# mycophonic/saprobe-alac

Hardware: AMD Instinct MI355X
Metric: Msamples/s decoded (16-bit stereo, 4096-frame packets) (higher is better)
Workload: dtype int32; 1 GPU; 65536 packets/GPU x 16-bit 2-ch 4096-frame ALAC, music-like synthetic, device-resident in/out; packets_per_gpu=65536

## Files before the change

### saprobe-alac_amd/csrc/alac_gpu.h

```cpp
#ifndef ALAC_GPU_H
#define ALAC_GPU_H
#include <hip/hip_runtime.h>

#include <algorithm>
#include <cstdio>
#include <cstdlib>
#include <cstring>

#define ALAC_DEV __device__ __forceinline__
#define ALAC_HD __host__ __device__ __forceinline__
#define ALAC_NOINLINE
#define ALAC_MUL24(a, b) __mul24((int)(a), (int)(b))
__device__ __forceinline__ uint32_t alac_sad(uint32_t a, uint32_t b, uint32_t c) {
    uint32_t r;
    asm("v_sad_u32 %0, %1, %2, %3" : "=v"(r) : "v"(a), "v"(b), "v"(c));
    return r;
}
#define ALAC_SAD(a, b, c) alac_sad((uint32_t)(a), (uint32_t)(b), (uint32_t)(c))

__device__ __forceinline__ int32_t alac_sign_med3(int32_t x) {
    int32_t r;
    asm("v_med3_i32 %0, %1, -1, 1" : "=v"(r) : "v"(x));
    return r;
}
// ... 102 lines not shown
#include "alac_duo.h"
#include "alac_split.h"

#define ALAC_PRIO_B_LONG 3
#define ALAC_PRIO_B_MID 2
#define ALAC_PRIO_B_SHORT 1
#define ALAC_PRIO_A 2
#define ALAC_PRIO_C 3

namespace alack {


typedef uint32_t u32x4 __attribute__((ext_vector_type(4)));

constexpr uint32_t kWave = 64;
constexpr uint32_t kTimingSlots = 64;
#ifndef ALAC_LDS_ROWS
#define ALAC_LDS_ROWS 64
#endif
#ifndef ALAC_LDS_RING
#define ALAC_LDS_RING 32
#endif
#ifndef ALAC_LDS_FLUSH
#define ALAC_LDS_FLUSH (ALAC_LDS_ROWS / 2)
#endif
constexpr uint32_t kRing = ALAC_LDS_ROWS;
constexpr uint32_t kFlush = ALAC_LDS_FLUSH;
static_assert(kFlush <= kRing && kRing % 4 == 0 && (kFlush == 16 || kFlush == 32), "the stager flushes 64- or 128-byte pieces of its rows");
constexpr uint32_t kRowStride = kRing + 1;
constexpr uint32_t kFallbackSlots = 64;
constexpr uint32_t kRingDw = ALAC_LDS_RING;
constexpr uint32_t kRingSlots = kRingDw + 2;

constexpr uint32_t kKeys = alac::KEY_IRREGULAR + 2u;
constexpr uint32_t kKeyLegacy = alac::KEY_IRREGULAR;
constexpr uint32_t kKeyScan = alac::KEY_IRREGULAR + 1u;
struct Plan {
    uint32_t count[kKeys];
    uint32_t pkt_start[kKeys];
    uint32_t cursor[kKeys];
    uint32_t nk;
    uint32_t list_key[kKeys];
    uint32_t list_wave0[kKeys];
    uint32_t total_waves;
    uint32_t irr_waves;
    uint32_t wide_waves;
    uint32_t gate[2][512];
    uint32_t balance[2][512];
    uint32_t queue[2];
};

static __shared__ uint32_t s_rows[kWave * kRowStride];
static __shared__ unsigned long long s_optr[kWave];
static __shared__ __attribute__((aligned(16))) uint32_t s_ring[kRingSlots * kWave];
constexpr uint32_t kQ = alac::DUO_CHUNK;
static __shared__ int32_t s_rq[2 * kQ * kWave];

#ifdef ALAC_SYNC_DIAG
constexpr uint32_t kClaimDw = 16;
static __shared__ uint32_t s_dg_arrive;
#else
constexpr uint32_t kClaimDw = 4;
#endif

__host__ __device__ inline size_t u_tile_cells(uint32_t frame_length) { return ((size_t)frame_length + 1u) * kWave; }

struct GpuWave {
    static constexpr bool kResMem = false;
    static constexpr uint32_t kRingDw = alack::kRingDw;
    int32_t* u_tile;
    int32_t* g_tile;
    uint8_t* my_out;
    uint32_t lane, wcnt, flushed;
    uint32_t ppw;
#ifdef ALAC_SYNC_DIAG
    uint32_t dg_wait[2] = {0, 0}, dg_last[2] = {0, 0};
    uint32_t dg_phase = 0, dg_waves = 3;
#endif

    ALAC_DEV bool any(bool p) const { return __ballot(p) != 0ull; }
    ALAC_DEV uint32_t max_u32(uint32_t v) const {
#pragma unroll
// ... 144 lines not shown
        asm volatile("s_waitcnt lgkmcnt(0)\n\ts_barrier" ::: "memory");
        dg_wait[dg_phase] += (uint32_t)(__builtin_amdgcn_s_memtime() - t0);
        dg_last[dg_phase] += (old + 1u) % dg_waves == 0u ? 1u : 0u;
    }
#endif
    ALAC_DEV void duo_sync_mem() {
        __threadfence_block();
        __syncthreads();
    }
    ALAC_DEV int32_t* u_row(uint32_t i) const { return u_tile + ((size_t)i * kWave + (ppw < kWave ? (lane < ppw ? lane : ppw) : lane)); }
    ALAC_DEV int32_t* g_slot(uint32_t k) const { return g_tile + (size_t)k * ppw; }
};

struct GpuWaveMem : GpuWave {
    static constexpr bool kResMem = true;
    const int32_t* res;
    uint32_t it, chunk0;
    ALAC_DEV int32_t rq_read(uint32_t, uint32_t j) const { return res[chunk0 + j]; }
    ALAC_DEV void rq_write(uint32_t, uint32_t, int32_t) {}
    ALAC_DEV void duo_sync() {
        ++it;
        chunk0 = (it - 1u) * kQ;
    }
    ALAC_DEV void duo_sync_mem() {}
};

__device__ __forceinline__ uint32_t avail_of(uint64_t blob_bytes, uint64_t off) {
    const uint64_t left = blob_bytes - off;
    return left > 0xffffffffull ? 0xffffffffu : (uint32_t)left;
}

__global__ void alac_classify(alac::DevCfg cfg, const uint8_t* __restrict__ blob, uint64_t blob_bytes, const uint64_t* __restrict__ offsets,
                              const uint32_t* __restrict__ sizes, uint32_t n, uint16_t* __restrict__ keys, uint32_t* __restrict__ sizes_ws,
                              uint32_t* __restrict__ frames_out, int32_t* __restrict__ status, Plan* plan);
__global__ void alac_plan(Plan* plan, uint32_t ppw);
__global__ void alac_cu_census(uint32_t* __restrict__ seen, uint32_t* __restrict__ arrived, uint32_t expect);
__global__ void alac_scatter(const uint16_t* __restrict__ keys, uint32_t n, Plan* plan, uint32_t* __restrict__ perm);
__global__ void alac_task_classify(alac::DevCfg cfg, const alac::ChanDesc* __restrict__ cd, const alac::PktDesc* __restrict__ pd,
                                   const uint16_t* __restrict__ pkt_keys, uint32_t n_slots, uint16_t* __restrict__ keys, Plan* plan);
__global__ void alac_scan(alac::DevCfg cfg, const uint8_t* __restrict__ blob, uint64_t blob_bytes, const uint64_t* __restrict__ offsets,
                          const uint32_t* __restrict__ sizes, const uint32_t* __restrict__ perm, const Plan* __restrict__ plan,
                          uint8_t* __restrict__ out, uint64_t out_stride, uint32_t* __restrict__ frames_out,
                          int32_t* __restrict__ status, int32_t* __restrict__ scratch_u, int32_t* __restrict__ scratch_g,
                          uint32_t ppw, alac::ChanDesc* __restrict__ cd, alac::PktDesc* __restrict__ pd, int32_t* __restrict__ rows,
                          uint64_t row_stride);
__global__ void alac_legacy(alac::DevCfg cfg, const uint8_t* __restrict__ blob, uint64_t blob_bytes, const uint64_t* __restrict__ offsets,
                            const uint32_t* __restrict__ sizes, const uint32_t* __restrict__ perm, const Plan* __restrict__ plan,
                            const alac::PktDesc* __restrict__ pd, uint8_t* __restrict__ out, uint64_t out_stride,
                            uint32_t* __restrict__ frames_out, int32_t* __restrict__ status, int32_t* __restrict__ scratch_u,
                            int32_t* __restrict__ scratch_g, uint32_t ppw);
constexpr uint32_t kModeFit4 = 4u, kModeFit5 = 5u, kModeGated = 6u;
constexpr __host__ __device__ __forceinline__ uint32_t decode_mode(uint32_t items, uint32_t n_cu, uint32_t cap, uint32_t force, bool mono,
                                                                  bool fit5) {
    if (force == kModeFit4 || (force == kModeFit5 && fit5)) return force;
    if (items <= 4u * n_cu) return kModeFit4;
    if (items <= 5u * n_cu) return (cap >= 5u && !mono) ? kModeGated : fit5 ? kModeFit5 : kModeFit4;
    if (items <= 6u * n_cu && cap >= 6u) return kModeGated;
    return (2u * items <= 15u * n_cu || !fit5) ? kModeFit4 : kModeFit5;
}
constexpr __host__ __device__ __forceinline__ uint32_t pair_quota(uint32_t items, uint32_t n_cu, uint32_t cap) {
    const uint32_t need = (items + n_cu - 1u) / n_cu;
    return need < 5u ? 5u : need < cap ? need : cap;
}
constexpr bool mode_is_fit4_without_the_others(uint32_t n_cu) {
    for (uint32_t items = 0u; items <= 40u * n_cu; items += (items < 8u * n_cu ? 1u : n_cu / 2u + 1u))
        if (decode_mode(items, n_cu, 0u, 0u, false, false) != kModeFit4 || decode_mode(items, n_cu, 0u, 5u, true, false) != kModeFit4) return false;
    return true;
}
constexpr bool mode_is_fit4_within_four(uint32_t n_cu) {
    for (uint32_t cap = 0u; cap <= 8u; ++cap)
        for (uint32_t items = 0u; items <= 4u * n_cu; ++items)
            if (decode_mode(items, n_cu, cap, 0u, false, true) != kModeFit4 || decode_mode(items, n_cu, cap, 0u, true, true) != kModeFit4) return false;
// ... 50 lines not shown
```

### saprobe-alac_amd/csrc/alacgpu.hip

```cpp
#include "alac_gpu.h"
#include "alac_host.h"
#include "alac_waveform.h"
#include "alac_clips.h"

using namespace alack;

namespace {
thread_local char g_err[512] = "";
}

void alack::set_err(const char* fmt, ...) {
    va_list ap;
    va_start(ap, fmt);
    vsnprintf(g_err, sizeof(g_err), fmt, ap);
    va_end(ap);
}

namespace {

class CopyPool {
public:
    explicit CopyPool(unsigned threads) {
        for (unsigned t = 0; t < threads; ++t) workers_.emplace_back([this] { run(); });
    }
    ~CopyPool() {
        {
            std::lock_guard<std::mutex> g(m_);
            stop_ = true;
        }
        cv_.notify_all();
        for (auto& w : workers_) w.join();
    }
// ... 90 lines not shown
Kernels choose_kernels(const alac::DevCfg& c) {
    Kernels k{};
    k.lean = alac::lean_config(c);
    k.one_or_two = c.num_channels <= 2;
    k.quad = c.bit_depth == 16 ? ALAC_PAIR_KERNEL(alac_decode_16q) : c.bit_depth == 32 ? ALAC_PAIR_KERNEL(alac_decode_32q) : ALAC_PAIR_KERNEL(alac_decode_24q);
    k.gated = c.bit_depth == 16 ? ALAC_PAIR_KERNEL(alac_decode_16g) : PairKernel{nullptr, ""};
    k.wide = c.bit_depth == 32 ? ALAC_PAIR_KERNEL(alac_decode_w32) : c.bit_depth == 24 ? ALAC_PAIR_KERNEL(alac_decode_w24) : PairKernel{nullptr, ""};
    const bool four_frames = c.num_channels > 2 && (c.num_channels * c.bps) % 4u == 0u;
    k.interleave = four_frames ? alac_interleave4 : alac_interleave;
    k.interleave_lds = (four_frames ? 128u : 32u) * kWave;
    k.irregular = !k.lean        ? "alac_scan (whole-packet decoder)"
                  : k.one_or_two ? "alac_scan + alac_interleave (+ alac_legacy)"
                  : four_frames  ? "alac_scan + alac_chan_predict + alac_interleave4 (+ alac_legacy)"
                                 : "alac_scan + alac_chan_predict + alac_interleave (+ alac_legacy)";
    return k;
}
#undef ALAC_PAIR_KERNEL

}

struct alacgpu_decoder {
    alacgpu_config cfg;
    alac::DevCfg dev_cfg;
    Kernels kernels;
    int device;
    size_t frame_bytes;
    hipStream_t stream;
    hipStream_t s_in, s_out;
    hipStream_t s_side;
    hipEvent_t ev_fork, ev_join;
    hipEvent_t ev_start[kTimingSlots], ev_stop[kTimingSlots];
    uint64_t launches;
    DevBuf scratch_u, scratch_g, plan, cls, perm, sizes_ws;
    DevBuf cd, pd, plan2, keys2, perm2, rows;
    Slot slots[kSlots];
    CopyPool* pool;
    uint32_t n_cu;
    DevBuf cu_number;
    size_t chunk_bytes;
    uint32_t lanes_min;
    int side;
    std::thread* ahead;
    int ahead_rc;
    char ahead_err[512];
    size_t last_n;
    uint32_t last_ppw, last_cap, last_fit5;
    uint32_t fit_force;
    DevBuf wave_ws;
    hipEvent_t ev_w0, ev_w1;
    bool wave_timed;
    hipEvent_t ev_c0, ev_c1;
    bool clips_timed;
};

namespace {

size_t plan_claims_offset() { return (sizeof(Plan) + 255u) & ~(size_t)255u; }
size_t plan_bytes(size_t waves) { return plan_claims_offset() + waves * kClaimDw * sizeof(uint32_t); }

struct KernelAttr {
    uint32_t pairs_per_cu, static_lds;
};
KernelAttr kernel_attr(void (*kernel)(PairArgs)) {
    static std::mutex mu;
    static std::vector<std::pair<const void*, KernelAttr>> cache;
    std::lock_guard<std::mutex> g(mu);
// ... 21 lines not shown
    HIP_TRY(hipMemcpyAsync(seen, dec->cu_number.p, sizeof(seen), hipMemcpyDeviceToHost, dec->stream));
    HIP_TRY(hipStreamSynchronize(dec->stream));
    uint32_t per_xcd[8] = {0}, xcds = 0, total = 0;
    for (uint32_t i = 0; i < 512; i++)
        if (seen[i]) {
            per_xcd[i >> 6]++;
            total++;
        }
    for (uint32_t x = 0; x < 8; x++) xcds += per_xcd[x] ? 1u : 0u;
    if (xcds == 0) xcds = 1;
    uint32_t next[8] = {0}, order[8] = {0}, k = 0;
    for (uint32_t x = 0; x < 8; x++)
        if (per_xcd[x]) order[x] = k++;
    for (uint32_t i = 0; i < 512; i++)
        if (seen[i]) {
            const uint32_t x = i >> 6;
            seen[i] = 1u + next[x]++ * xcds + order[x];
        }
    if (total > dec->n_cu) dec->n_cu = total;
    HIP_TRY(hipMemcpyAsync(dec->cu_number.p, seen, sizeof(seen), hipMemcpyHostToDevice, dec->stream));
    HIP_TRY(hipStreamSynchronize(dec->stream));
    return ALACGPU_E_OK;
}

size_t max_waves(uint32_t bit_depth, size_t n, uint32_t ppw) {
    const size_t keys = (bit_depth >= 24 ? 2 : 1) * 18 * 18 + 8;
    return (n + ppw - 1) / ppw + std::min<size_t>(n, keys);
}
size_t max_waves(const alacgpu_decoder* dec, size_t n, uint32_t ppw) { return max_waves(dec->cfg.bit_depth, n, ppw); }

uint32_t pick_ppw(size_t n) {
    if (const char* e = getenv("ALACGPU_PPW")) {
        const int v = atoi(e);
        if (v >= 1 && v <= 64) return (uint32_t)v;
    }
    uint32_t ppw = kWave;
    while (ppw > 1 && n / ppw < 256) ppw >>= 1;
    return ppw;
}

size_t row_stride_of(uint32_t frame_length) { return ((size_t)frame_length + 3u) & ~(size_t)3u; }

int reserve_workspace(alacgpu_decoder* dec, size_t n, uint32_t ppw) {
    const size_t waves = max_waves(dec, n, ppw);
    int rc;
    if ((rc = dec->scratch_u.ensure(waves * u_tile_cells(dec->cfg.frame_length) * sizeof(int32_t)))) return rc;
    if ((rc = dec->scratch_g.ensure(waves * kFallbackSlots * ppw * sizeof(int32_t)))) return rc;
    if ((rc = dec->plan.ensure(plan_bytes(waves)))) return rc;
    if ((rc = dec->cls.ensure((n ? n : 1) * sizeof(uint16_t)))) return rc;
    if ((rc = dec->perm.ensure((n ? n : 1) * sizeof(uint32_t)))) return rc;
    if ((rc = dec->sizes_ws.ensure((n ? n : 1) * sizeof(uint32_t)))) return rc;
    const size_t ns = (n ? n : 1) * 8;
    if ((rc = dec->cd.ensure(ns * sizeof(alac::ChanDesc)))) return rc;
    if ((rc = dec->pd.ensure((n ? n : 1) * sizeof(alac::PktDesc)))) return rc;
    if (dec->cfg.num_channels > 2) {
        if ((rc = dec->plan2.ensure(sizeof(Plan)))) return rc;
        if ((rc = dec->keys2.ensure(ns * sizeof(uint16_t)))) return rc;
        if ((rc = dec->perm2.ensure(ns * sizeof(uint32_t)))) return rc;
        if ((rc = dec->rows.ensure((n ? n : 1) * dec->cfg.num_channels * row_stride_of(dec->cfg.frame_length) * sizeof(int32_t))))
            return rc;
    }
    return ALACGPU_E_OK;
}

struct Launch {
    alacgpu_decoder* dec;
    alac::DevCfg c;
    const uint8_t* d_blob;
    uint64_t blob_bytes;
    const uint64_t* d_offsets;
    size_t n;
    uint8_t* d_out;
    size_t out_stride;
    uint32_t* d_frames;
    int32_t* d_status;
    uint32_t ppw;
    size_t waves;
    hipStream_t irr;
    bool forked;
    uint32_t scan_grid;
    Plan* plan() const { return (Plan*)dec->plan.p; }
    const uint32_t* sz() const { return (const uint32_t*)dec->sizes_ws.p; }
};

struct SideFork {
    alacgpu_decoder* dec;
    bool open = false;
    int fork() {
        HIP_TRY(hipEventRecord(dec->ev_fork, dec->stream));
        HIP_TRY(hipStreamWaitEvent(dec->s_side, dec->ev_fork, 0));
        open = true;
        return ALACGPU_E_OK;
    }
    int join() {
        HIP_TRY(hipEventRecord(dec->ev_join, dec->s_side));
        HIP_TRY(hipStreamWaitEvent(dec->stream, dec->ev_join, 0));
        open = false;
        return ALACGPU_E_OK;
    }
    ~SideFork() {
        if (open) (void)hipStreamSynchronize(dec->s_side);
    }
};

int sort_pass(const Launch& L, const uint32_t* d_sizes) {
    alacgpu_decoder* dec = L.dec;
    const uint32_t nb = (uint32_t)((L.n + 255) / 256);
    HIP_TRY(hipMemsetAsync(L.plan(), 0, plan_bytes(L.waves), dec->stream));
    hipLaunchKernelGGL(alac_classify, dim3(nb), dim3(256), 0, dec->stream, L.c, L.d_blob, L.blob_bytes, L.d_offsets, d_sizes,
                       (uint32_t)L.n, (uint16_t*)dec->cls.p, (uint32_t*)dec->sizes_ws.p, L.d_frames, L.d_status, L.plan());
    hipLaunchKernelGGL(alac_plan, dim3(1), dim3(kWave), 0, dec->stream, L.plan(), L.ppw);
    hipLaunchKernelGGL(alac_scatter, dim3(nb), dim3(256), 0, dec->stream, (const uint16_t*)dec->cls.p, (uint32_t)L.n, L.plan(),
                       (uint32_t*)dec->perm.p);
    return ALACGPU_E_OK;
}

void scan(const Launch& L) {
    alacgpu_decoder* dec = L.dec;
    hipLaunchKernelGGL(alac_scan, dim3(L.scan_grid), dim3(kWave), 0, L.irr, L.c, L.d_blob, L.blob_bytes,
                       L.d_offsets, L.sz(), (const uint32_t*)dec->perm.p, (const Plan*)L.plan(), L.d_out, (uint64_t)L.out_stride, L.d_frames,
                       L.d_status, (int32_t*)dec->scratch_u.p, (int32_t*)dec->scratch_g.p, L.ppw, (alac::ChanDesc*)dec->cd.p,
                       (alac::PktDesc*)dec->pd.p, dec->cfg.num_channels > 2 ? (int32_t*)dec->rows.p : (int32_t*)nullptr,
                       (uint64_t)row_stride_of(dec->cfg.frame_length));
}

void narrow_launch(const Launch& L, const PairArgs& a, uint32_t slots, uint32_t mode) {
    alacgpu_decoder* dec = L.dec;
    const Kernels& k = dec->kernels;
    if (mode == kModeGated) {
        if (a.cap) hipLaunchKernelGGL(k.gated.fn, dim3(std::min<uint32_t>(a.cap * dec->n_cu, slots)), dim3(2 * kWave), 0, dec->stream, a);
        return;
    }
    if (mode == kModeFit5 && !a.fit5) return;
    const uint32_t stat = kernel_attr(k.quad.fn).static_lds;
    PairArgs q = a;
    q.fit = mode;
    hipLaunchKernelGGL(k.quad.fn, dim3(slots), dim3(4 * kWave), (mode == kModeFit4 && stat < kQuadLdsFit4) ? kQuadLdsFit4 - stat : 0u,
                       dec->stream, q);
}

void regular_packets(const Launch& L) {
    alacgpu_decoder* dec = L.dec;
    const Kernels& k = dec->kernels;
    const size_t n = L.n;
    const uint32_t ppw = L.ppw;
    PairArgs a{L.c, L.d_blob, (uint64_t)L.blob_bytes, L.d_offsets, L.sz(), (const uint32_t*)dec->perm.p, L.plan(), L.d_out, (uint64_t)L.out_stride,
               L.d_frames, L.d_status, (int32_t*)dec->scratch_u.p, (const uint32_t*)dec->cu_number.p,
               (uint32_t*)((uint8_t*)L.plan() + plan_claims_offset()), ppw, dec->n_cu, 0u, dec->lanes_min, 4u, dec->fit_force, 0u};
    const uint32_t slots = (uint32_t)L.waves;
    const uint32_t n_cu = dec->n_cu;
    const bool beyond4 = (n + ppw - 1) / ppw > (size_t)4 * n_cu || dec->fit_force == kModeFit5;
    const bool has_twin = k.gated.fn && beyond4 && dec->fit_force == 0u;
    {
        const uint32_t stat = kernel_attr(k.quad.fn).static_lds;
        a.fit5 = (beyond4 && (size_t)((stat + 1279u) / 1280u) * 1280u * 5u <= 163840u) ? 1u : 0u;
    }
    if (has_twin) a.cap = kernel_attr(k.gated.fn).pairs_per_cu;
    if (a.cap <= 4u) a.cap = 0u;
    dec->last_cap = a.cap;
    dec->last_fit5 = a.fit5;
    const uint32_t guess = decode_mode((uint32_t)((n + ppw - 1) / ppw), n_cu, a.cap, dec->fit_force, dec->cfg.num_channels == 1, a.fit5 != 0u);
    narrow_launch(L, a, slots, guess);
    if (k.wide.fn) hipLaunchKernelGGL(k.wide.fn, dim3(slots), dim3(2 * kWave), 0, dec->stream, a);
    for (uint32_t mode : {kModeFit4, kModeFit5, kModeGated})
        if (mode != guess) narrow_launch(L, a, slots, mode);
}

int split_pipeline(const Launch& L) {
    alacgpu_decoder* dec = L.dec;
    Plan* plan2 = (Plan*)dec->plan2.p;
    const size_t n_slots = L.n * 8;
    const uint32_t nb2 = (uint32_t)((n_slots + 255) / 256);
    const uint32_t ppw2 = pick_ppw(L.n * dec->cfg.num_channels);
    HIP_TRY(hipMemsetAsync(plan2, 0, sizeof(Plan), dec->stream));
    hipLaunchKernelGGL(alac_task_classify, dim3(nb2), dim3(256), 0, dec->stream, L.c, (const alac::ChanDesc*)dec->cd.p,
                       (const alac::PktDesc*)dec->pd.p, (const uint16_t*)dec->cls.p, (uint32_t)n_slots,
                       (uint16_t*)dec->keys2.p, plan2);
    hipLaunchKernelGGL(alac_plan, dim3(1), dim3(kWave), 0, dec->stream, plan2, ppw2);
    hipLaunchKernelGGL(alac_scatter, dim3(nb2), dim3(256), 0, dec->stream, (const uint16_t*)dec->keys2.p,
                       (uint32_t)n_slots, plan2, (uint32_t*)dec->perm2.p);
    hipLaunchKernelGGL(alac_chan_predict, dim3((uint32_t)max_waves(16u, n_slots, ppw2)), dim3(kWave), 0, dec->stream, L.c,
                       L.d_blob, L.blob_bytes, L.d_offsets, L.sz(), (const uint32_t*)dec->perm2.p, (const Plan*)plan2,
                       (const alac::ChanDesc*)dec->cd.p, (int32_t*)dec->rows.p, (uint64_t)row_stride_of(dec->cfg.frame_length), ppw2);
    return ALACGPU_E_OK;
}

void irregular_pcm(const Launch& L) {
    alacgpu_decoder* dec = L.dec;
    const Kernels& k = dec->kernels;
    const uint64_t rs = row_stride_of(dec->cfg.frame_length);
    const uint32_t bpp = (dec->cfg.frame_length + kWave - 1u) / kWave;
    const uint32_t ib = (uint32_t)std::min<uint64_t>((uint64_t)L.n * ((bpp + 7u) / 8u), L.forked ? (uint64_t)4 * dec->n_cu : (uint64_t)32768u);
    hipLaunchKernelGGL(k.interleave, dim3(ib), dim3(kWave), k.interleave_lds, L.irr, L.c, L.d_blob, L.blob_bytes, L.d_offsets, L.sz(),
                       (const uint32_t*)dec->perm.p, (const Plan*)L.plan(), (const alac::ChanDesc*)dec->cd.p,
                       (const alac::PktDesc*)dec->pd.p, (const int32_t*)dec->rows.p, rs, L.d_out, (uint64_t)L.out_stride, bpp);
    hipLaunchKernelGGL(alac_legacy, dim3(L.scan_grid), dim3(kWave), 0, L.irr, L.c, L.d_blob, L.blob_bytes,
                       L.d_offsets, L.sz(), (const uint32_t*)dec->perm.p, (const Plan*)L.plan(), (const alac::PktDesc*)dec->pd.p, L.d_out,
                       (uint64_t)L.out_stride, L.d_frames, L.d_status, (int32_t*)dec->scratch_u.p, (int32_t*)dec->scratch_g.p, L.ppw);
}

int launch(alacgpu_decoder* dec, const uint8_t* d_blob, uint64_t blob_bytes, const uint64_t* d_offsets,
           const uint32_t* d_sizes, size_t n, uint8_t* d_out, size_t out_stride, uint32_t* d_frames, int32_t* d_status) {
    if (n == 0) return ALACGPU_E_OK;
    if (n > 0x7fffffffu) {
        set_err("batch too large");
        return ALACGPU_E_ARG;
    }
    const uint32_t ppw = pick_ppw(n);
    int rc = reserve_workspace(dec, n, ppw);
    if (rc) return rc;
    dec->last_n = n;
    dec->last_ppw = ppw;
    dec->last_cap = dec->last_fit5 = 0;
    const Kernels& k = dec->kernels;
    Launch L{dec, dec->dev_cfg, d_blob, blob_bytes, d_offsets, n, d_out, out_stride, d_frames, d_status, ppw, max_waves(dec, n, ppw),
             dec->stream, false, 0u};
    L.c.aligned16 = (out_stride % 16 == 0 && (reinterpret_cast<uintptr_t>(d_out) % 16) == 0) ? 1u : 0u;
    const uint32_t slot = (uint32_t)(dec->launches % kTimingSlots);
    HIP_TRY(hipEventRecord(dec->ev_start[slot], dec->stream));
    if ((rc = sort_pass(L, d_sizes))) return rc;
    L.forked = k.one_or_two && k.lean &&
               (dec->side >= 2 || (dec->side == 1 && (n + ppw - 1) / ppw <= (size_t)6 * dec->n_cu));
    L.scan_grid = (uint32_t)std::min<size_t>(L.waves, (size_t)(L.forked ? 2u : 6u) * dec->n_cu);
    SideFork side{dec};
    if (L.forked) {
        if ((rc = side.fork())) return rc;
        L.irr = dec->s_side;
    }
    if (!L.forked) scan(L);
    if (k.one_or_two && k.lean) regular_packets(L);
    if (L.forked) scan(L);
    HIP_TRY(hipGetLastError());
    if (k.lean) {
        if (!k.one_or_two && (rc = split_pipeline(L))) return rc;
        irregular_pcm(L);
        HIP_TRY(hipGetLastError());
    }
    if (L.forked && (rc = side.join())) return rc;
    HIP_TRY(hipEventRecord(dec->ev_stop[slot], dec->stream));
    dec->launches++;
    return ALACGPU_E_OK;
}

}

namespace {
std::mutex g_pool_mu;
std::vector<alacgpu_decoder*> g_pool;
std::vector<std::pair<void*, size_t>> g_host_pool;
std::vector<std::pair<void*, size_t>> g_host_sizes;
constexpr size_t kPoolPerDevice = 4;
constexpr size_t kPoolKeepDevice = (size_t)2048 << 20;
constexpr size_t kPoolKeepPinned = (size_t)64 << 20;
constexpr size_t kHostPoolBlock = (size_t)64 << 20, kHostPoolBytes = (size_t)192 << 20, kHostPoolCount = 8;
template <class Buf>
void keep_at_most(std::vector<Buf*> bufs, size_t limit) {
    for (;;) {
        size_t total = 0;
        Buf* big = nullptr;
        for (Buf* b : bufs) {
            total += b->cap;
            if (b->cap && (!big || b->cap > big->cap)) big = b;
        }
        if (total <= limit || !big) return;
        big->release();
    }
}

std::vector<DevBuf*> device_buffers(alacgpu_decoder* d) {
    std::vector<DevBuf*> v = {&d->scratch_u, &d->scratch_g, &d->plan, &d->cls, &d->perm, &d->sizes_ws, &d->cd, &d->pd,
                              &d->plan2, &d->keys2, &d->perm2, &d->rows, &d->wave_ws};
    for (Slot& s : d->slots) v.insert(v.end(), {&s.d_in, &s.d_out});
    return v;
}
std::vector<HostBuf*> pinned_buffers(alacgpu_decoder* d) {
    std::vector<HostBuf*> v;
    for (Slot& s : d->slots) v.insert(v.end(), {&s.h_in, &s.h_out});
    return v;
}
std::vector<hipStream_t*> streams_of(alacgpu_decoder* d) { return {&d->stream, &d->s_in, &d->s_out, &d->s_side}; }
struct EventRef {
    hipEvent_t* ev;
    unsigned flags;
};
std::vector<EventRef> events_of(alacgpu_decoder* d) {
    std::vector<EventRef> v = {{&d->ev_fork, hipEventDisableTiming}, {&d->ev_join, hipEventDisableTiming},
                               {&d->ev_w0, hipEventDefault}, {&d->ev_w1, hipEventDefault},
                               {&d->ev_c0, hipEventDefault}, {&d->ev_c1, hipEventDefault}};
    for (uint32_t i = 0; i < kTimingSlots; i++) v.insert(v.end(), {{&d->ev_start[i], hipEventDefault}, {&d->ev_stop[i], hipEventDefault}});
    for (Slot& s : d->slots)
        v.insert(v.end(), {{&s.ev_in, hipEventDisableTiming}, {&s.ev_k, hipEventDisableTiming}, {&s.ev_out, hipEventDisableTiming}});
    return v;
}

bool synchronize_all(alacgpu_decoder* d) {
    bool ok = true;
    for (hipStream_t* s : streams_of(d))
        if (*s && hipStreamSynchronize(*s) != hipSuccess) ok = false;
    return ok;
}

void really_destroy(alacgpu_decoder* d) {
    (void)hipSetDevice(d->device);
// ... 79 lines not shown
        return ALACGPU_E_ARG;
    }
    d->device = device;
    configure(d, cfg);
    {
        int cus = 0;
        if (hipDeviceGetAttribute(&cus, hipDeviceAttributeMultiprocessorCount, device) != hipSuccess) cus = 0;
        d->n_cu = cus > 0 ? (uint32_t)cus : 256u;
    }
    hipError_t e = hipSuccess;
    for (hipStream_t* st : streams_of(d))
        if (e == hipSuccess) e = hipStreamCreateWithFlags(st, hipStreamNonBlocking);
    for (const EventRef& ev : events_of(d))
        if (e == hipSuccess) e = hipEventCreateWithFlags(ev.ev, ev.flags);
    if (e != hipSuccess) {
        set_err("stream/event creation failed: %s", hipGetErrorString(e));
        really_destroy(d);
        return ALACGPU_E_HIP;
    }
    if (int rc = cu_numbers(d)) {
        really_destroy(d);
        return rc;
    }
    *out = d;
    return ALACGPU_E_OK;
}

void alacgpu_destroy(alacgpu_decoder* d) {
    if (!d) return;
    (void)settle_ahead(d);
    (void)hipSetDevice(d->device);
    if (synchronize_all(d)) {
        for (int k = 0; k < kSlots; k++) d->slots[k].busy = false;
        keep_at_most(device_buffers(d), kPoolKeepDevice);
        keep_at_most(pinned_buffers(d), kPoolKeepPinned);
        std::lock_guard<std::mutex> g(g_pool_mu);
        size_t same = 0;
        for (alacgpu_decoder* p : g_pool) same += p->device == d->device ? 1u : 0u;
        if (same < kPoolPerDevice) {
            g_pool.push_back(d);
            return;
        }
    }
    really_destroy(d);
}

void alacgpu_trim(void) {
    std::vector<alacgpu_decoder*> all;
    std::vector<std::pair<void*, size_t>> host;
    {
        std::lock_guard<std::mutex> g(g_pool_mu);
        all.swap(g_pool);
        host.swap(g_host_pool);
    }
    for (alacgpu_decoder* d : all) really_destroy(d);
    for (auto& h : host) (void)hipHostFree(h.first);
}

void* alacgpu_host_alloc(size_t bytes) {
    if (bytes == 0) bytes = 1;
    {
        std::lock_guard<std::mutex> g(g_pool_mu);
        size_t best = SIZE_MAX;
        for (size_t i = 0; i < g_host_pool.size(); i++)
            if (g_host_pool[i].second >= bytes && g_host_pool[i].second <= 2 * bytes + (1u << 20) &&
                (best == SIZE_MAX || g_host_pool[i].second < g_host_pool[best].second))
// ... 513 lines not shown
```

### saprobe-alac_amd/csrc/k_sort.hip

```cpp
#include "alac_gpu.h"

namespace alack {

__global__ void __launch_bounds__(256)
alac_classify(alac::DevCfg cfg, const uint8_t* __restrict__ blob, uint64_t blob_bytes, const uint64_t* __restrict__ offsets,
              const uint32_t* __restrict__ sizes, uint32_t n, uint16_t* __restrict__ keys, uint32_t* __restrict__ sizes_ws,
              uint32_t* __restrict__ frames_out, int32_t* __restrict__ status, Plan* plan) {
    __shared__ uint32_t hist[kKeys];
    for (uint32_t k = threadIdx.x; k < kKeys; k += blockDim.x) hist[k] = 0;
    __syncthreads();
    const uint32_t i = blockIdx.x * blockDim.x + threadIdx.x;
    if (i < n) {
        const uint64_t off = offsets[i];
        uint64_t sz = sizes ? (uint64_t)sizes[i] : offsets[i + 1] - off;
        const bool ok = off <= blob_bytes && sz <= blob_bytes - off && sz <= 0x0fffffffull &&
                        (sizes || offsets[i + 1] >= off);
        if (!ok) {
            keys[i] = (uint16_t)alac::TASK_NONE;
            sizes_ws[i] = 0;
            frames_out[i] = 0;
            status[i] = ALACGPU_ERR_RANGE;
        } else if (sz == 0) {
            keys[i] = (uint16_t)alac::TASK_NONE;
            sizes_ws[i] = 0;
            frames_out[i] = 0;
            status[i] = ALACGPU_STATUS(alac::ST_OVERRUN, 0, 0);
        } else {
            sizes_ws[i] = (uint32_t)sz;
            const uint8_t* p = blob + off;
            uint32_t key = alac::classify_regular(cfg, p, (uint32_t)sz, avail_of(blob_bytes, off));
            if (key == alac::KEY_IRREGULAR) key = alac::lean_config(cfg) ? kKeyScan : kKeyLegacy;
            keys[i] = (uint16_t)key;
            atomicAdd(&hist[key], 1u);
        }
    }
    __syncthreads();
    for (uint32_t k = threadIdx.x; k < kKeys; k += blockDim.x)
        if (hist[k]) atomicAdd(&plan->count[k], hist[k]);
}

__global__ void __launch_bounds__(kWave) alac_plan(Plan* plan, uint32_t ppw) {
    __shared__ uint32_t cnt[kKeys];
    for (uint32_t k = threadIdx.x; k < kKeys; k += kWave) cnt[k] = plan->count[k];
    __syncthreads();
    constexpr uint32_t R = (kKeys + kWave - 1) / kWave;
    const uint32_t q0 = threadIdx.x * R;
    uint32_t p = 0, w = 0, z = 0, wi = 0, ww = 0;
    for (uint32_t r = 0; r < R; ++r) {
        const uint32_t q = q0 + r;
        if (q >= kKeys) break;
        const uint32_t key = kKeys - 1u - q;
        const uint32_t c = cnt[key];
        const uint32_t cw = (c + ppw - 1) / ppw;
        p += c;
        w += cw;
        z += c ? 1u : 0u;
        wi += key >= alac::KEY_IRREGULAR ? cw : 0u;
        ww += (key >= alac::KEY_WIDE && key < alac::KEY_IRREGULAR) ? cw : 0u;
    }
    uint32_t ip = p, iw = w, iz = z, ii = wi, ix = ww;
#pragma unroll
    for (int o = 1; o < (int)kWave; o <<= 1) {
        const uint32_t tp = (uint32_t)__shfl_up((int)ip, o, kWave), tw = (uint32_t)__shfl_up((int)iw, o, kWave);
        const uint32_t tz = (uint32_t)__shfl_up((int)iz, o, kWave), ti = (uint32_t)__shfl_up((int)ii, o, kWave);
        const uint32_t tx = (uint32_t)__shfl_up((int)ix, o, kWave);
        if ((int)threadIdx.x >= o) {
            ix += tx;
            ip += tp;
            iw += tw;
            iz += tz;
            ii += ti;
        }
    }
    uint32_t ep = ip - p, ew = iw - w, ez = iz - z;
    for (uint32_t r = 0; r < R; ++r) {
        const uint32_t q = q0 + r;
        if (q >= kKeys) break;
        const uint32_t key = kKeys - 1u - q;
        const uint32_t c = cnt[key];
        plan->pkt_start[key] = ep;
        plan->cursor[key] = 0;
        if (c) {
            plan->list_key[ez] = key;
            plan->list_wave0[ez] = ew;
            ++ez;
            ep += c;
            ew += (c + ppw - 1) / ppw;
        }
    }
    if (threadIdx.x == kWave - 1u) {
        plan->nk = iz;
        plan->total_waves = iw;
        plan->irr_waves = ii;
        plan->wide_waves = ix;
    }
}

__global__ void __launch_bounds__(256)
alac_scatter(const uint16_t* __restrict__ keys, uint32_t n, Plan* plan, uint32_t* __restrict__ perm) {
    __shared__ uint32_t hist[kKeys];
    __shared__ uint32_t base[kKeys];
    for (uint32_t k = threadIdx.x; k < kKeys; k += blockDim.x) hist[k] = 0;
    __syncthreads();
    const uint32_t i = blockIdx.x * blockDim.x + threadIdx.x;
    uint32_t key = 0, local = 0;
    if (i < n) {
        key = keys[i];
        if (key != alac::TASK_NONE) local = atomicAdd(&hist[key], 1u);
    }
    __syncthreads();
    for (uint32_t k = threadIdx.x; k < kKeys; k += blockDim.x)
        if (hist[k]) base[k] = plan->pkt_start[k] + atomicAdd(&plan->cursor[k], hist[k]);
    __syncthreads();
    if (i < n && key != alac::TASK_NONE) perm[base[key] + local] = i;
}

__global__ void __launch_bounds__(256)
alac_task_classify(alac::DevCfg cfg, const alac::ChanDesc* __restrict__ cd, const alac::PktDesc* __restrict__ pd,
                   const uint16_t* __restrict__ pkt_keys, uint32_t n_slots, uint16_t* __restrict__ keys, Plan* plan) {
    __shared__ uint32_t hist[alac::NUM_TASK_KEYS];
    if (threadIdx.x < alac::NUM_TASK_KEYS) hist[threadIdx.x] = 0;
    __syncthreads();
    const uint32_t t = blockIdx.x * blockDim.x + threadIdx.x;
    if (t < n_slots) {
        const uint32_t pkt = t >> 3, slot = t & 7u;
        uint32_t key = alac::TASK_NONE;
        if (pkt_keys[pkt] == kKeyScan) {
            const alac::PktDesc q = pd[pkt];
            if (q.status == 0 && q.route == alac::ROUTE_SPLIT && slot < q.nslots) {
                const alac::ChanDesc d = cd[t];
                if ((d.info & alac::CD_VALID) && !(d.info & alac::CD_ESCAPE)) key = alac::chan_task_key(cfg, d);
            }
        }
        keys[t] = (uint16_t)key;
        if (key != alac::TASK_NONE) atomicAdd(&hist[key], 1u);
    }
    __syncthreads();
    if (threadIdx.x < alac::NUM_TASK_KEYS && hist[threadIdx.x]) atomicAdd(&plan->count[threadIdx.x], hist[threadIdx.x]);
}

__global__ void __launch_bounds__(kWave) alac_cu_census(uint32_t* __restrict__ seen, uint32_t* __restrict__ arrived, uint32_t expect) {
    __shared__ uint32_t pad[16384];
    pad[threadIdx.x] = threadIdx.x;
    if (threadIdx.x == 0) {
        uint32_t id, xcc;
        asm volatile("s_getreg_b32 %0, hwreg(HW_REG_HW_ID)" : "=s"(id));
        asm volatile("s_getreg_b32 %0, hwreg(HW_REG_XCC_ID)" : "=s"(xcc));
        seen[((xcc & 7u) << 6) | (((id >> 13) & 3u) << 4) | ((id >> 8) & 15u)] = 1u;
        atomicAdd(arrived, 1u);
        for (int i = 0; i < 4000 && atomicAdd(arrived, 0u) < expect; ++i) __builtin_amdgcn_s_sleep(32);
    }
    __syncthreads();
    if (pad[(threadIdx.x * 5u) & 63u] == 0xffffffffu) seen[0] = 2u;
}

}
```

Before: 264,200 Msamples/s.

## Fuse plan computation into classify via last-block ticket and rank-based scatter

```diff
diff --git a/saprobe-alac_amd/csrc/alac_gpu.h b/saprobe-alac_amd/csrc/alac_gpu.h
--- a/saprobe-alac_amd/csrc/alac_gpu.h
+++ b/saprobe-alac_amd/csrc/alac_gpu.h
@@ -158,22 +158,13 @@
 constexpr uint32_t kRingDw = ALAC_LDS_RING;
 constexpr uint32_t kRingSlots = kRingDw + 2;
 
-constexpr uint32_t kKeys = alac::KEY_IRREGULAR + 2u;
-constexpr uint32_t kKeyLegacy = alac::KEY_IRREGULAR;
-constexpr uint32_t kKeyScan = alac::KEY_IRREGULAR + 1u;
-struct Plan {
-    uint32_t count[kKeys];
-    uint32_t pkt_start[kKeys];
-    uint32_t cursor[kKeys];
-    uint32_t nk;
-    uint32_t list_key[kKeys];
-    uint32_t list_wave0[kKeys];
-    uint32_t total_waves;
-    uint32_t irr_waves;
-    uint32_t wide_waves;
-    uint32_t gate[2][512];
-    uint32_t balance[2][512];
-    uint32_t queue[2];
+}
+#include "alac_plan.h"
+namespace alack {
+
+struct SortWs {
+    uint32_t hist[kKeys];
+    uint32_t ticket;
 };
 
 static __shared__ uint32_t s_rows[kWave * kRowStride];
@@ -384,12 +375,14 @@
 
 __global__ void alac_classify(alac::DevCfg cfg, const uint8_t* __restrict__ blob, uint64_t blob_bytes, const uint64_t* __restrict__ offsets,
                               const uint32_t* __restrict__ sizes, uint32_t n, uint16_t* __restrict__ keys, uint32_t* __restrict__ sizes_ws,
-                              uint32_t* __restrict__ frames_out, int32_t* __restrict__ status, Plan* plan);
-__global__ void alac_plan(Plan* plan, uint32_t ppw);
+                              uint32_t* __restrict__ frames_out, int32_t* __restrict__ status, uint32_t* __restrict__ rank, SortWs* ws, Plan* plan,
+                              uint32_t ppw_shift);
 __global__ void alac_cu_census(uint32_t* __restrict__ seen, uint32_t* __restrict__ arrived, uint32_t expect);
-__global__ void alac_scatter(const uint16_t* __restrict__ keys, uint32_t n, Plan* plan, uint32_t* __restrict__ perm);
+__global__ void alac_scatter(const uint16_t* __restrict__ keys, const uint32_t* __restrict__ rank, uint32_t n, const Plan* __restrict__ plan,
+                             uint32_t* __restrict__ perm, uint32_t* __restrict__ claims, uint32_t claim_dw);
 __global__ void alac_task_classify(alac::DevCfg cfg, const alac::ChanDesc* __restrict__ cd, const alac::PktDesc* __restrict__ pd,
-                                   const uint16_t* __restrict__ pkt_keys, uint32_t n_slots, uint16_t* __restrict__ keys, Plan* plan);
+                                   const uint16_t* __restrict__ pkt_keys, uint32_t n_slots, uint16_t* __restrict__ keys, uint32_t* __restrict__ rank,
+                                   SortWs* ws, Plan* plan, uint32_t ppw_shift);
 __global__ void alac_scan(alac::DevCfg cfg, const uint8_t* __restrict__ blob, uint64_t blob_bytes, const uint64_t* __restrict__ offsets,
                           const uint32_t* __restrict__ sizes, const uint32_t* __restrict__ perm, const Plan* __restrict__ plan,
                           uint8_t* __restrict__ out, uint64_t out_stride, uint32_t* __restrict__ frames_out,
diff --git a/saprobe-alac_amd/csrc/alac_plan.h b/saprobe-alac_amd/csrc/alac_plan.h
--- /dev/null
+++ b/saprobe-alac_amd/csrc/alac_plan.h
@@ -0,0 +1,72 @@
+#ifndef ALAC_PLAN_H
+#define ALAC_PLAN_H
+#include <stdint.h>
+
+#ifndef ALAC_DEV
+#error "define ALAC_DEV before including alac_plan.h"
+#endif
+
+namespace alack {
+
+constexpr uint32_t kKeys = alac::KEY_IRREGULAR + 2u;
+constexpr uint32_t kKeyLegacy = alac::KEY_IRREGULAR;
+constexpr uint32_t kKeyScan = alac::KEY_IRREGULAR + 1u;
+struct Plan {
+    uint32_t count[kKeys];
+    uint32_t pkt_start[kKeys];
+    uint32_t spare[kKeys];
+    uint32_t nk;
+    uint32_t list_key[kKeys];
+    uint32_t list_wave0[kKeys];
+    uint32_t total_waves;
+    uint32_t irr_waves;
+    uint32_t wide_waves;
+    uint32_t gate[2][512];
+    uint32_t balance[2][512];
+    uint32_t queue[2];
+};
+constexpr uint32_t kPlanZeroDw = 2u * 512u + 2u * 512u + 2u;
+
+struct PlanSums {
+    uint32_t pkts, waves, keys, irr, wide;
+};
+ALAC_DEV uint32_t plan_waves_of(uint32_t c, uint32_t shift) { return (c + (1u << shift) - 1u) >> shift; }
+ALAC_DEV PlanSums plan_run_sums(const uint32_t* cnt, uint32_t q0, uint32_t run, uint32_t shift) {
+    PlanSums s{0u, 0u, 0u, 0u, 0u};
+    for (uint32_t q = q0; q < q0 + run && q < kKeys; ++q) {
+        const uint32_t key = kKeys - 1u - q;
+        const uint32_t c = cnt[key];
+        const uint32_t cw = plan_waves_of(c, shift);
+        s.pkts += c;
+        s.waves += cw;
+        s.keys += c ? 1u : 0u;
+        s.irr += key >= alac::KEY_IRREGULAR ? cw : 0u;
+        s.wide += (key >= alac::KEY_WIDE && key < alac::KEY_IRREGULAR) ? cw : 0u;
+    }
+    return s;
+}
+ALAC_DEV void plan_run_emit(const uint32_t* cnt, uint32_t q0, uint32_t run, uint32_t shift, PlanSums before, Plan* plan) {
+    uint32_t ep = before.pkts, ew = before.waves, ez = before.keys;
+    for (uint32_t q = q0; q < q0 + run && q < kKeys; ++q) {
+        const uint32_t key = kKeys - 1u - q;
+        const uint32_t c = cnt[key];
+        plan->count[key] = c;
+        plan->pkt_start[key] = ep;
+        if (c) {
+            plan->list_key[ez] = key;
+            plan->list_wave0[ez] = ew;
+            ++ez;
+            ep += c;
+            ew += plan_waves_of(c, shift);
+        }
+    }
+}
+ALAC_DEV void plan_totals(PlanSums all, Plan* plan) {
+    plan->nk = all.keys;
+    plan->total_waves = all.waves;
+    plan->irr_waves = all.irr;
+    plan->wide_waves = all.wide;
+}
+
+}
+#endif
diff --git a/saprobe-alac_amd/csrc/alacgpu.hip b/saprobe-alac_amd/csrc/alacgpu.hip
--- a/saprobe-alac_amd/csrc/alacgpu.hip
+++ b/saprobe-alac_amd/csrc/alacgpu.hip
@@ -1,3 +1,5 @@
+#include <cassert>
+
 #include "alac_gpu.h"
 #include "alac_host.h"
 #include "alac_waveform.h"
@@ -154,6 +156,8 @@
     hipEvent_t ev_start[kTimingSlots], ev_stop[kTimingSlots];
     uint64_t launches;
     DevBuf scratch_u, scratch_g, plan, cls, perm, sizes_ws;
+    DevBuf rank, sort_ws;
+    bool sort_dirty;
     DevBuf cd, pd, plan2, keys2, perm2, rows;
     Slot slots[kSlots];
     CopyPool* pool;
@@ -241,11 +245,15 @@
 uint32_t pick_ppw(size_t n) {
     if (const char* e = getenv("ALACGPU_PPW")) {
         const int v = atoi(e);
-        if (v >= 1 && v <= 64) return (uint32_t)v;
+        if (v >= 1 && v <= 64 && (v & (v - 1)) == 0) return (uint32_t)v;
     }
     uint32_t ppw = kWave;
     while (ppw > 1 && n / ppw < 256) ppw >>= 1;
     return ppw;
+}
+uint32_t ppw_shift_of(uint32_t ppw) {
+    assert(ppw >= 1u && ppw <= kWave && (ppw & (ppw - 1u)) == 0u);
+    return (uint32_t)__builtin_ctz(ppw);
 }
 
 size_t row_stride_of(uint32_t frame_length) { return ((size_t)frame_length + 3u) & ~(size_t)3u; }
@@ -256,10 +264,16 @@
     if ((rc = dec->scratch_u.ensure(waves * u_tile_cells(dec->cfg.frame_length) * sizeof(int32_t)))) return rc;
     if ((rc = dec->scratch_g.ensure(waves * kFallbackSlots * ppw * sizeof(int32_t)))) return rc;
     if ((rc = dec->plan.ensure(plan_bytes(waves)))) return rc;
+    if (!dec->sort_ws.p) {
+        if ((rc = dec->sort_ws.ensure(sizeof(SortWs)))) return rc;
+        HIP_TRY(hipMemsetAsync(dec->sort_ws.p, 0, sizeof(SortWs), dec->stream));
+        dec->sort_dirty = false;
+    }
     if ((rc = dec->cls.ensure((n ? n : 1) * sizeof(uint16_t)))) return rc;
     if ((rc = dec->perm.ensure((n ? n : 1) * sizeof(uint32_t)))) return rc;
     if ((rc = dec->sizes_ws.ensure((n ? n : 1) * sizeof(uint32_t)))) return rc;
     const size_t ns = (n ? n : 1) * 8;
+    if ((rc = dec->rank.ensure((dec->cfg.num_channels > 2 ? ns : (n ? n : 1)) * sizeof(uint32_t)))) return rc;
     if ((rc = dec->cd.ensure(ns * sizeof(alac::ChanDesc)))) return rc;
     if ((rc = dec->pd.ensure((n ? n : 1) * sizeof(alac::PktDesc)))) return rc;
     if (dec->cfg.num_channels > 2) {
@@ -315,12 +329,15 @@
 int sort_pass(const Launch& L, const uint32_t* d_sizes) {
     alacgpu_decoder* dec = L.dec;
     const uint32_t nb = (uint32_t)((L.n + 255) / 256);
-    HIP_TRY(hipMemsetAsync(L.plan(), 0, plan_bytes(L.waves), dec->stream));
+    if (dec->sort_dirty) HIP_TRY(hipMemsetAsync(dec->sort_ws.p, 0, sizeof(SortWs), dec->stream));
+    dec->sort_dirty = true;
     hipLaunchKernelGGL(alac_classify, dim3(nb), dim3(256), 0, dec->stream, L.c, L.d_blob, L.blob_bytes, L.d_offsets, d_sizes,
-                       (uint32_t)L.n, (uint16_t*)dec->cls.p, (uint32_t*)dec->sizes_ws.p, L.d_frames, L.d_status, L.plan());
-    hipLaunchKernelGGL(alac_plan, dim3(1), dim3(kWave), 0, dec->stream, L.plan(), L.ppw);
-    hipLaunchKernelGGL(alac_scatter, dim3(nb), dim3(256), 0, dec->stream, (const uint16_t*)dec->cls.p, (uint32_t)L.n, L.plan(),
-                       (uint32_t*)dec->perm.p);
+                       (uint32_t)L.n, (uint16_t*)dec->cls.p, (uint32_t*)dec->sizes_ws.p, L.d_frames, L.d_status, (uint32_t*)dec->rank.p,
+                       (SortWs*)dec->sort_ws.p, L.plan(), ppw_shift_of(L.ppw));
+    HIP_TRY(hipGetLastError());
+    hipLaunchKernelGGL(alac_scatter, dim3(nb), dim3(256), 0, dec->stream, (const uint16_t*)dec->cls.p, (const uint32_t*)dec->rank.p,
+                       (uint32_t)L.n, (const Plan*)L.plan(), (uint32_t*)dec->perm.p, (uint32_t*)((uint8_t*)L.plan() + plan_claims_offset()),
+                       (uint32_t)(L.waves * kClaimDw));
     return ALACGPU_E_OK;
 }
 
@@ -381,13 +398,12 @@
     const size_t n_slots = L.n * 8;
     const uint32_t nb2 = (uint32_t)((n_slots + 255) / 256);
     const uint32_t ppw2 = pick_ppw(L.n * dec->cfg.num_channels);
-    HIP_TRY(hipMemsetAsync(plan2, 0, sizeof(Plan), dec->stream));
     hipLaunchKernelGGL(alac_task_classify, dim3(nb2), dim3(256), 0, dec->stream, L.c, (const alac::ChanDesc*)dec->cd.p,
                        (const alac::PktDesc*)dec->pd.p, (const uint16_t*)dec->cls.p, (uint32_t)n_slots,
-                       (uint16_t*)dec->keys2.p, plan2);
-    hipLaunchKernelGGL(alac_plan, dim3(1), dim3(kWave), 0, dec->stream, plan2, ppw2);
-    hipLaunchKernelGGL(alac_scatter, dim3(nb2), dim3(256), 0, dec->stream, (const uint16_t*)dec->keys2.p,
-                       (uint32_t)n_slots, plan2, (uint32_t*)dec->perm2.p);
+                       (uint16_t*)dec->keys2.p, (uint32_t*)dec->rank.p, (SortWs*)dec->sort_ws.p, plan2, ppw_shift_of(ppw2));
+    HIP_TRY(hipGetLastError());
+    hipLaunchKernelGGL(alac_scatter, dim3(nb2), dim3(256), 0, dec->stream, (const uint16_t*)dec->keys2.p, (const uint32_t*)dec->rank.p,
+                       (uint32_t)n_slots, (const Plan*)plan2, (uint32_t*)dec->perm2.p, (uint32_t*)nullptr, 0u);
     hipLaunchKernelGGL(alac_chan_predict, dim3((uint32_t)max_waves(16u, n_slots, ppw2)), dim3(kWave), 0, dec->stream, L.c,
                        L.d_blob, L.blob_bytes, L.d_offsets, L.sz(), (const uint32_t*)dec->perm2.p, (const Plan*)plan2,
                        (const alac::ChanDesc*)dec->cd.p, (int32_t*)dec->rows.p, (uint64_t)row_stride_of(dec->cfg.frame_length), ppw2);
@@ -448,6 +464,7 @@
     if (L.forked && (rc = side.join())) return rc;
     HIP_TRY(hipEventRecord(dec->ev_stop[slot], dec->stream));
     dec->launches++;
+    dec->sort_dirty = false;
     return ALACGPU_E_OK;
 }
 
@@ -477,7 +494,7 @@
 }
 
 std::vector<DevBuf*> device_buffers(alacgpu_decoder* d) {
-    std::vector<DevBuf*> v = {&d->scratch_u, &d->scratch_g, &d->plan, &d->cls, &d->perm, &d->sizes_ws, &d->cd, &d->pd,
+    std::vector<DevBuf*> v = {&d->scratch_u, &d->scratch_g, &d->plan, &d->cls, &d->perm, &d->sizes_ws, &d->rank, &d->sort_ws, &d->cd, &d->pd,
                               &d->plan2, &d->keys2, &d->perm2, &d->rows, &d->wave_ws};
     for (Slot& s : d->slots) v.insert(v.end(), {&s.d_in, &s.d_out});
     return v;
@@ -623,6 +640,8 @@
     (void)hipSetDevice(d->device);
     if (synchronize_all(d)) {
         for (int k = 0; k < kSlots; k++) d->slots[k].busy = false;
+        if (d->sort_dirty) d->sort_ws.release();
+        d->sort_dirty = false;
         keep_at_most(device_buffers(d), kPoolKeepDevice);
         keep_at_most(pinned_buffers(d), kPoolKeepPinned);
         std::lock_guard<std::mutex> g(g_pool_mu);
diff --git a/saprobe-alac_amd/csrc/k_sort.hip b/saprobe-alac_amd/csrc/k_sort.hip
--- a/saprobe-alac_amd/csrc/k_sort.hip
+++ b/saprobe-alac_amd/csrc/k_sort.hip
@@ -2,129 +2,138 @@
 
 namespace alack {
 
+#define ALAC_RLX_AGENT __ATOMIC_RELAXED, __HIP_MEMORY_SCOPE_AGENT
+
+__device__ __forceinline__ void sort_reserve(uint32_t* hist, uint32_t used, SortWs* ws) {
+    __syncthreads();
+    for (uint32_t k = threadIdx.x; k < used; k += blockDim.x) {
+        const uint32_t c = hist[k];
+        if (c) hist[k] = __hip_atomic_fetch_add(&ws->hist[k], c, ALAC_RLX_AGENT);
+    }
+    __syncthreads();
+}
+
+__device__ __forceinline__ void sort_finish(uint32_t* hist, SortWs* ws, Plan* plan, uint32_t ppw_shift) {
+    __shared__ uint32_t s_last;
+    __shared__ uint32_t s_wave[4][5];
+    __syncthreads();
+    if (threadIdx.x == 0) s_last = __hip_atomic_fetch_add(&ws->ticket, 1u, ALAC_RLX_AGENT) == gridDim.x - 1u ? 1u : 0u;
+    __syncthreads();
+    if (!s_last) return;
+    constexpr uint32_t R = (kKeys + 255u) / 256u;
+    {
+        uint32_t c[R];
+#pragma unroll
+        for (uint32_t r = 0; r < R; ++r) {
+            const uint32_t k = threadIdx.x + r * 256u;
+            c[r] = k < kKeys ? __hip_atomic_load(&ws->hist[k], ALAC_RLX_AGENT) : 0u;
+        }
+        if (threadIdx.x == 0) __hip_atomic_store(&ws->ticket, 0u, ALAC_RLX_AGENT);
+        uint32_t* z = &plan->gate[0][0];
+        for (uint32_t k = threadIdx.x; k < kPlanZeroDw; k += 256u) z[k] = 0u;
+#pragma unroll
+        for (uint32_t r = 0; r < R; ++r) {
+            const uint32_t k = threadIdx.x + r * 256u;
+            if (k < kKeys) hist[k] = c[r];
+            if (c[r]) __hip_atomic_store(&ws->hist[k], 0u, ALAC_RLX_AGENT);
+        }
+    }
+    __syncthreads();
+    const uint32_t q0 = threadIdx.x * R;
+    const PlanSums own = plan_run_sums(hist, q0, R, ppw_shift);
+    uint32_t v[5] = {own.pkts, own.waves, own.keys, own.irr, own.wide};
+    const uint32_t lane = threadIdx.x & (kWave - 1u), wave = threadIdx.x / kWave;
+#pragma unroll
+    for (int o = 1; o < (int)kWave; o <<= 1) {
+#pragma unroll
+        for (int j = 0; j < 5; ++j) {
+            const uint32_t t = (uint32_t)__shfl_up((int)v[j], o, kWave);
+            if ((int)lane >= o) v[j] += t;
+        }
+    }
+    if (lane == kWave - 1u)
+        for (int j = 0; j < 5; ++j) s_wave[wave][j] = v[j];
+    __syncthreads();
+    uint32_t all[5];
+#pragma unroll
+    for (int j = 0; j < 5; ++j) {
+        uint32_t front = 0, total = 0;
+        for (uint32_t w = 0; w < 4u; ++w) {
+            front += w < wave ? s_wave[w][j] : 0u;
+            total += s_wave[w][j];
+        }
+        v[j] += front;
+        all[j] = total;
+    }
+    plan_run_emit(hist, q0, R, ppw_shift, PlanSums{v[0] - own.pkts, v[1] - own.waves, v[2] - own.keys, v[3] - own.irr, v[4] - own.wide}, plan);
+    if (threadIdx.x == 0) plan_totals(PlanSums{all[0], all[1], all[2], all[3], all[4]}, plan);
+}
+static_assert(offsetof(Plan, queue) + sizeof(Plan::queue) - offsetof(Plan, gate) == kPlanZeroDw * sizeof(uint32_t) &&
+                  offsetof(Plan, queue) + sizeof(Plan::queue) == sizeof(Plan),
+              "gate, balance and queue are the tail of the plan, back to back");
+
 __global__ void __launch_bounds__(256)
 alac_classify(alac::DevCfg cfg, const uint8_t* __restrict__ blob, uint64_t blob_bytes, const uint64_t* __restrict__ offsets,
               const uint32_t* __restrict__ sizes, uint32_t n, uint16_t* __restrict__ keys, uint32_t* __restrict__ sizes_ws,
-              uint32_t* __restrict__ frames_out, int32_t* __restrict__ status, Plan* plan) {
+              uint32_t* __restrict__ frames_out, int32_t* __restrict__ status, uint32_t* __restrict__ rank, SortWs* ws, Plan* plan,
+              uint32_t ppw_shift) {
     __shared__ uint32_t hist[kKeys];
     for (uint32_t k = threadIdx.x; k < kKeys; k += blockDim.x) hist[k] = 0;
     __syncthreads();
     const uint32_t i = blockIdx.x * blockDim.x + threadIdx.x;
+    uint32_t key = alac::TASK_NONE, local = 0;
     if (i < n) {
         const uint64_t off = offsets[i];
         uint64_t sz = sizes ? (uint64_t)sizes[i] : offsets[i + 1] - off;
         const bool ok = off <= blob_bytes && sz <= blob_bytes - off && sz <= 0x0fffffffull &&
                         (sizes || offsets[i + 1] >= off);
         if (!ok) {
-            keys[i] = (uint16_t)alac::TASK_NONE;
             sizes_ws[i] = 0;
             frames_out[i] = 0;
             status[i] = ALACGPU_ERR_RANGE;
         } else if (sz == 0) {
-            keys[i] = (uint16_t)alac::TASK_NONE;
             sizes_ws[i] = 0;
             frames_out[i] = 0;
             status[i] = ALACGPU_STATUS(alac::ST_OVERRUN, 0, 0);
         } else {
             sizes_ws[i] = (uint32_t)sz;
             const uint8_t* p = blob + off;
-            uint32_t key = alac::classify_regular(cfg, p, (uint32_t)sz, avail_of(blob_bytes, off));
+            key = alac::classify_regular(cfg, p, (uint32_t)sz, avail_of(blob_bytes, off));
             if (key == alac::KEY_IRREGULAR) key = alac::lean_config(cfg) ? kKeyScan : kKeyLegacy;
-            keys[i] = (uint16_t)key;
-            atomicAdd(&hist[key], 1u);
+            local = atomicAdd(&hist[key], 1u);
         }
+        keys[i] = (uint16_t)key;
     }
-    __syncthreads();
-    for (uint32_t k = threadIdx.x; k < kKeys; k += blockDim.x)
-        if (hist[k]) atomicAdd(&plan->count[k], hist[k]);
+    sort_reserve(hist, kKeys, ws);
+    if (key != alac::TASK_NONE) rank[i] = hist[key] + local;
+    sort_finish(hist, ws, plan, ppw_shift);
 }
 
-__global__ void __launch_bounds__(kWave) alac_plan(Plan* plan, uint32_t ppw) {
-    __shared__ uint32_t cnt[kKeys];
-    for (uint32_t k = threadIdx.x; k < kKeys; k += kWave) cnt[k] = plan->count[k];
-    __syncthreads();
-    constexpr uint32_t R = (kKeys + kWave - 1) / kWave;
-    const uint32_t q0 = threadIdx.x * R;
-    uint32_t p = 0, w = 0, z = 0, wi = 0, ww = 0;
-    for (uint32_t r = 0; r < R; ++r) {
-        const uint32_t q = q0 + r;
-        if (q >= kKeys) break;
-        const uint32_t key = kKeys - 1u - q;
-        const uint32_t c = cnt[key];
-        const uint32_t cw = (c + ppw - 1) / ppw;
-        p += c;
-        w += cw;
-        z += c ? 1u : 0u;
-        wi += key >= alac::KEY_IRREGULAR ? cw : 0u;
-        ww += (key >= alac::KEY_WIDE && key < alac::KEY_IRREGULAR) ? cw : 0u;
-    }
-    uint32_t ip = p, iw = w, iz = z, ii = wi, ix = ww;
-#pragma unroll
-    for (int o = 1; o < (int)kWave; o <<= 1) {
-        const uint32_t tp = (uint32_t)__shfl_up((int)ip, o, kWave), tw = (uint32_t)__shfl_up((int)iw, o, kWave);
-        const uint32_t tz = (uint32_t)__shfl_up((int)iz, o, kWave), ti = (uint32_t)__shfl_up((int)ii, o, kWave);
-        const uint32_t tx = (uint32_t)__shfl_up((int)ix, o, kWave);
-        if ((int)threadIdx.x >= o) {
-            ix += tx;
-            ip += tp;
-            iw += tw;
-            iz += tz;
-            ii += ti;
+__global__ void __launch_bounds__(256)
+alac_scatter(const uint16_t* __restrict__ keys, const uint32_t* __restrict__ rank, uint32_t n, const Plan* __restrict__ plan,
+             uint32_t* __restrict__ perm, uint32_t* __restrict__ claims, uint32_t claim_dw) {
+    const uint32_t i = blockIdx.x * blockDim.x + threadIdx.x;
+    for (uint32_t k = i; k < claim_dw; k += gridDim.x * blockDim.x) claims[k] = 0u;
+    if (i < n) {
+        const uint32_t key = keys[i];
+        if (key != alac::TASK_NONE) {
+            const uint32_t at = plan->pkt_start[key] + rank[i];
+            if (at < n) perm[at] = i;
         }
-    }
-    uint32_t ep = ip - p, ew = iw - w, ez = iz - z;
-    for (uint32_t r = 0; r < R; ++r) {
-        const uint32_t q = q0 + r;
-        if (q >= kKeys) break;
-        const uint32_t key = kKeys - 1u - q;
-        const uint32_t c = cnt[key];
-        plan->pkt_start[key] = ep;
-        plan->cursor[key] = 0;
-        if (c) {
-            plan->list_key[ez] = key;
-            plan->list_wave0[ez] = ew;
-            ++ez;
-            ep += c;
-            ew += (c + ppw - 1) / ppw;
-        }
-    }
-    if (threadIdx.x == kWave - 1u) {
-        plan->nk = iz;
-        plan->total_waves = iw;
-        plan->irr_waves = ii;
-        plan->wide_waves = ix;
     }
 }
 
 __global__ void __launch_bounds__(256)
-alac_scatter(const uint16_t* __restrict__ keys, uint32_t n, Plan* plan, uint32_t* __restrict__ perm) {
+alac_task_classify(alac::DevCfg cfg, const alac::ChanDesc* __restrict__ cd, const alac::PktDesc* __restrict__ pd,
+                   const uint16_t* __restrict__ pkt_keys, uint32_t n_slots, uint16_t* __restrict__ keys, uint32_t* __restrict__ rank,
+                   SortWs* ws, Plan* plan, uint32_t ppw_shift) {
     __shared__ uint32_t hist[kKeys];
-    __shared__ uint32_t base[kKeys];
-    for (uint32_t k = threadIdx.x; k < kKeys; k += blockDim.x) hist[k] = 0;
-    __syncthreads();
-    const uint32_t i = blockIdx.x * blockDim.x + threadIdx.x;
-    uint32_t key = 0, local = 0;
-    if (i < n) {
-        key = keys[i];
-        if (key != alac::TASK_NONE) local = atomicAdd(&hist[key], 1u);
-    }
-    __syncthreads();
-    for (uint32_t k = threadIdx.x; k < kKeys; k += blockDim.x)
-        if (hist[k]) base[k] = plan->pkt_start[k] + atomicAdd(&plan->cursor[k], hist[k]);
-    __syncthreads();
-    if (i < n && key != alac::TASK_NONE) perm[base[key] + local] = i;
-}
-
-__global__ void __launch_bounds__(256)
-alac_task_classify(alac::DevCfg cfg, const alac::ChanDesc* __restrict__ cd, const alac::PktDesc* __restrict__ pd,
-                   const uint16_t* __restrict__ pkt_keys, uint32_t n_slots, uint16_t* __restrict__ keys, Plan* plan) {
-    __shared__ uint32_t hist[alac::NUM_TASK_KEYS];
     if (threadIdx.x < alac::NUM_TASK_KEYS) hist[threadIdx.x] = 0;
     __syncthreads();
     const uint32_t t = blockIdx.x * blockDim.x + threadIdx.x;
+    uint32_t key = alac::TASK_NONE, local = 0;
     if (t < n_slots) {
         const uint32_t pkt = t >> 3, slot = t & 7u;
-        uint32_t key = alac::TASK_NONE;
         if (pkt_keys[pkt] == kKeyScan) {
             const alac::PktDesc q = pd[pkt];
             if (q.status == 0 && q.route == alac::ROUTE_SPLIT && slot < q.nslots) {
@@ -133,11 +142,13 @@
             }
         }
         keys[t] = (uint16_t)key;
-        if (key != alac::TASK_NONE) atomicAdd(&hist[key], 1u);
+        if (key != alac::TASK_NONE) local = atomicAdd(&hist[key], 1u);
     }
-    __syncthreads();
-    if (threadIdx.x < alac::NUM_TASK_KEYS && hist[threadIdx.x]) atomicAdd(&plan->count[threadIdx.x], hist[threadIdx.x]);
+    sort_reserve(hist, alac::NUM_TASK_KEYS, ws);
+    if (key != alac::TASK_NONE) rank[t] = hist[key] + local;
+    sort_finish(hist, ws, plan, ppw_shift);
 }
+#undef ALAC_RLX_AGENT
 
 __global__ void __launch_bounds__(kWave) alac_cu_census(uint32_t* __restrict__ seen, uint32_t* __restrict__ arrived, uint32_t expect) {
     __shared__ uint32_t pad[16384];
```

Result: faster. 267,000 Msamples/s (median of 6 runs) (+1.1%).
